# preiter93/rustpde-mpi

Hardware: NVIDIA H100
Metric: Navier2D timesteps/sec (higher is better)
Workload: dtype f64

## Files before the change

rustpde_mpi_b200/csrc/b200pde.cu:

```cuda
#include "lane_kernel.cuh"
#include "gemm_f64.cuh"
#include "../../include/b200pde.h"

#include <cmath>
#include <cstdlib>
#include <cstdio>
#include <cstring>
#include <map>
#include <string>
#include <vector>
#include <algorithm>

static thread_local std::string g_err;
static int fail(int code, const std::string& msg) { g_err = msg; return code; }
#define CK(call)                                                                                   \
  do {                                                                                             \
    cudaError_t e_ = (call);                                                                       \
    if (e_ != cudaSuccess)                                                                         \
      return fail(B2_ERR_CUDA, std::string(#call) + ": " + cudaGetErrorString(e_));                \
  } while (0)
#define RET(call)                    \
  do {                               \
    int r_ = (call);                 \
    if (r_ != B2_OK) return r_;      \
// ... 171 lines not shown
  LuVecs r;
  r.fl.assign(n, 0.0); r.id.assign(n, 0.0); r.u1.assign(n, 0.0); r.u2.assign(n, 0.0);
  for (int i = 0; i < n; i++) {
    if (i >= 2) r.fl[i] = low[i - 2];
    r.id[i] = 1.0 / dia[i];
    if (i < n - 2) r.u1[i] = up1[i];
    if (i < n - 4) r.u2[i] = up2[i];
  }
  return r;
}

static std::vector<double> pdma_sweep(int n, const std::vector<double> (&d)[7], int L) {
  const std::vector<double>&l2 = d[0], &l1 = d[1], &d0 = d[2], &u1 = d[3], &u2 = d[4], &u3 = d[5], &u4 = d[6];
  std::vector<double> al(n, 0.0), be(n, 0.0), ga(n, 0.0), de(n, 0.0), ka(n, 0.0), mu(n, 0.0);
  for (int i = 0; i < n; i++) {
    const double l2i = i >= 2 ? l2[i - 2] : 0.0;
    ka[i] = (i >= 1 ? l1[i - 1] : 0.0) - (i >= 2 ? al[i - 2] * l2i : 0.0);
    mu[i] = d0[i] - (i >= 2 ? be[i - 2] * l2i : 0.0) - (i >= 1 ? al[i - 1] * ka[i] : 0.0);
    if (i + 1 < n) al[i] = (u1[i] - (i >= 2 ? ga[i - 2] * l2i : 0.0) - (i >= 1 ? be[i - 1] * ka[i] : 0.0)) / mu[i];
    if (i + 2 < n) be[i] = (u2[i] - (i >= 2 ? de[i - 2] * l2i : 0.0) - (i >= 1 ? ga[i - 1] * ka[i] : 0.0)) / mu[i];
    if (i + 3 < n) ga[i] = (u3[i] - (i >= 1 ? de[i - 1] * ka[i] : 0.0)) / mu[i];
    if (i + 4 < n) de[i] = u4[i] / mu[i];
  }
  std::vector<double> out((size_t)7 * L, 0.0);
  for (int i = 0; i < n; i++) {
    out[i] = i >= 2 ? l2[i - 2] : 0.0; out[(size_t)L + i] = ka[i]; out[(size_t)2 * L + i] = 1.0 / mu[i];
    out[(size_t)3 * L + i] = al[i]; out[(size_t)4 * L + i] = be[i]; out[(size_t)5 * L + i] = ga[i]; out[(size_t)6 * L + i] = de[i];
  }
  return out;
}

static std::map<const void*, const void*>& scan_of() { static std::map<const void*, const void*> m; return m; }

struct Base1 {
  int kind = 0, n = 0, m = 0;
  bool cheb = false, composite = false;
  bool cdn = false;
  bool c2c = false;
  int rows_phys = 0, rows_spec = 0, rows_ortho = 0;
  int N = 0;
  std::vector<double> s2;
  DVecD d_sten2, d_sten2s, d_s2, d_tfl, d_tid, d_tu1, d_bd, d_bu1, d_bu2, d_tw, d_tw2, d_isin;
  std::vector<double> ca, cb;
  DVecD d_dfwd, d_dbwd; bool dense_tr = false;
  DVecD d_ca, d_cb, d_pent; int pent_L = 0;
  DVecD d_s2_sc, d_bd_sc, d_bu1_sc, d_bu2_sc, d_sten2s_sc;

  double pv(int i, int off) const {
    const int r = i + 2;
    if (off == 0) return r == 2 ? 0.25 : 1.0 / (4.0 * r * (r - 1.0));
    if (off == 2) return (r < n - 2) ? -1.0 / (2.0 * ((double)r * r - 1.0)) : 0.0;
    if (off == 4) return (r < n - 4) ? 1.0 / (4.0 * r * (r + 1.0)) : 0.0;
    return 0.0;
  }
  Diags mat_a() const {
    Diags a(m);
    for (int i = 0; i < m; i++) {
      if (i >= 2) a.low[i - 2] = pv(i, 0) * s2[i - 2];
      a.dia[i] = pv(i, 0) + pv(i, 2) * s2[i];
      if (i + 2 < m) a.up1[i] = pv(i, 2) + pv(i, 4) * s2[i + 2];
      if (i + 4 < m) a.up2[i] = pv(i, 4);
    }
    return a;
  }
  Diags mat_b() const {
    Diags b(m);
    for (int i = 0; i < m; i++) {
      b.dia[i] = s2[i];
      if (i + 2 < m) b.up1[i] = 1.0;
    }
    return b;
  }
  void cdn_hholtz_diags(double c, std::vector<double> (&d)[7]) const {
    auto S = [&](int r, int j) -> double { if (j < 0 || j >= m) return 0.0; return r == j ? 1.0 : (r == j + 1 ? ca[j] : (r == j + 2 ? cb[j] : 0.0)); };
    for (int k = 0; k < 7; k++) d[k].assign(m, 0.0);
    for (int i = 0; i < m; i++)
      for (int off = -2; off <= 4; off++) {
        const int j = i + off;
        if (j < 0 || j >= m) continue;
        const double a = pv(i, 0) * S(i, j) + pv(i, 2) * S(i + 2, j) + pv(i, 4) * S(i + 4, j);
        const double v = a - c * S(i + 2, j);
        d[off + 2][off >= 0 ? i : j] = v;
      }
  }
  int init_host(int kind_, int n_);
  int init(int C, int TPL);
  int lay_C = 1, lay_TPL = 1;
  std::vector<double> scan_layout(const std::vector<double>& v) const {
    std::vector<double> o((size_t)2 * lay_C * lay_TPL, 0.0);
    for (int q = 0; q < lay_TPL; q++)
      for (int t = 0; t < lay_C; t++) {
        const size_t p = (size_t)q * lay_C + t, k = (size_t)t * lay_TPL + q;
        if (2 * p < v.size()) o[2 * k] = v[2 * p];
        if (2 * p + 1 < v.size()) o[2 * k + 1] = v[2 * p + 1];
      }
    return o;
  }
  void release() {
    const void* keys[] = {d_bd.d, d_bu1.d, d_bu2.d, d_s2.d, d_sten2s.d};
    for (auto k : keys) if (k) scan_of().erase(k);
    DVecD* all[] = {&d_sten2, &d_sten2s, &d_s2, &d_tfl, &d_tid, &d_tu1, &d_bd, &d_bu1, &d_bu2, &d_tw, &d_tw2, &d_isin, &d_s2_sc, &d_bd_sc, &d_bu1_sc, &d_bu2_sc, &d_sten2s_sc, &d_ca, &d_cb, &d_pent, &d_dfwd, &d_dbwd};
    for (auto* v : all) v->release();
  }
};

static bool is_pow2(int x) { return x > 0 && (x & (x - 1)) == 0; }

int Base1::init_host(int kind_, int n_) {
  kind = kind_; n = n_;
  cheb = (kind <= B2_CHEB_DIRICHLET_NEUMANN);
  composite = (kind == B2_CHEB_DIRICHLET || kind == B2_CHEB_NEUMANN);
  cdn = (kind == B2_CHEB_DIRICHLET_NEUMANN);
  c2c = (kind == B2_FOURIER_C2C);
  if (kind < 0 || kind > B2_FOURIER_C2C) return fail(B2_ERR_ARG, "bad base kind");
  if (n < 5) return fail(B2_ERR_ARG, "n too small");
  if (cheb) {
    m = (composite || cdn) ? n - 2 : n;
    rows_phys = n; rows_spec = m; rows_ortho = n; N = n - 1;
  } else if (c2c) {
    if (n > 1024) return fail(B2_ERR_UNSUPPORTED, "fourier_c2c: n <= 1024 (dense-matrix transform)");
    m = n;
    rows_phys = 2 * n; rows_spec = 2 * n; rows_ortho = 2 * n; N = 0;
  } else {
    if (n % 2) return fail(B2_ERR_UNSUPPORTED, "fourier_r2c needs even n");
    m = n / 2 + 1;
    rows_phys = n; rows_spec = 2 * m; rows_ortho = 2 * m; N = n;
  }
  if (cdn) {
    ca.assign(m, 0.0); cb.assign(m, 0.0);
    for (int k = 0; k < m; k++) { const double kd = k; ca[k] = ((kd + 2) * (kd + 2) - kd * kd) / ((kd + 1) * (kd + 1) + (kd + 2) * (kd + 2)); cb[k] = ca[k] - 1.0; }
  }
  if (composite) {
    s2.assign(m, 0.0);
    for (int k = 0; k < m; k++) s2[k] = (kind == B2_CHEB_DIRICHLET) ? -1.0 : -((double)k / (k + 2.0)) * ((double)k / (k + 2.0));
  }
  return B2_OK;
}

int Base1::init(int C, int TPL) {
  lay_C = C; lay_TPL = TPL;
  const int L = roundup(std::max(rows_phys, rows_ortho) + 8, 4) + 64;
  if (composite) {
    std::vector<double> sten2(L, 0.0), s2v(L, 0.0);
    for (int i = 2; i < n; i++) sten2[i] = s2[i - 2];
    for (int k = 0; k < m; k++) s2v[k] = s2[k];
    RET(d_sten2.upload(sten2)); RET(d_sten2s.upload(sten2)); RET(d_s2.upload(s2v));
    Diags t(m);
    for (int k = 0; k < m; k++) {
      t.dia[k] = 1.0 + s2[k] * s2[k];
      if (k + 2 < m) { t.low[k] = s2[k]; t.up1[k] = s2[k]; }
    }
    LuVecs lu = sweep(t);
    lu.fl.resize(L, 0.0); lu.id.resize(L, 0.0); lu.u1.resize(L, 0.0);
    RET(d_tfl.upload(scan_layout(lu.fl))); RET(d_tid.upload(scan_layout(lu.id))); RET(d_tu1.upload(scan_layout(lu.u1)));
    std::vector<double> bd(L, 0.0), bu1(L, 0.0), bu2(L, 0.0);
    for (int i = 0; i < m; i++) {
      bd[i] = pv(i, 0);
      if (i < m - 2) bu1[i] = pv(i, 2);
      if (i < m - 4) bu2[i] = pv(i, 4);
    }
    RET(d_bd.upload(bd)); RET(d_bu1.upload(bu1)); RET(d_bu2.upload(bu2));
    RET(d_bd_sc.upload(scan_layout(bd))); RET(d_bu1_sc.upload(scan_layout(bu1))); RET(d_bu2_sc.upload(scan_layout(bu2))); RET(d_s2_sc.upload(scan_layout(s2v)));
    scan_of()[d_bd.d] = d_bd_sc.d; scan_of()[d_bu1.d] = d_bu1_sc.d; scan_of()[d_bu2.d] = d_bu2_sc.d; scan_of()[d_s2.d] = d_s2_sc.d;
    RET(d_sten2s_sc.upload(scan_layout(sten2))); scan_of()[d_sten2s.d] = d_sten2s_sc.d;
  }
  if (cdn) {
    std::vector<double> a(L, 0.0), b(L, 0.0);
    for (int k = 0; k < m; k++) { a[k] = ca[k]; b[k] = cb[k]; }
    RET(d_ca.upload(a)); RET(d_cb.upload(b));
    std::vector<double> d[7];
    for (int k = 0; k < 7; k++) d[k].assign(m, 0.0);
    for (int j = 0; j < m; j++) {
      d[2][j] = 1.0 + ca[j] * ca[j] + cb[j] * cb[j];
      if (j + 1 < m) { d[3][j] = ca[j] + cb[j] * ca[j + 1]; d[1][j] = d[3][j]; }
      if (j + 2 < m) { d[4][j] = cb[j]; d[0][j] = cb[j]; }
    }
    pent_L = L;
    RET(d_pent.upload(pdma_sweep(m, d, L)));
    std::vector<double> bd(L, 0.0), bu1(L, 0.0), bu2(L, 0.0);
    for (int i = 0; i < m; i++) {
      bd[i] = pv(i, 0);
      if (i < m - 2) bu1[i] = pv(i, 2);
      if (i < m - 4) bu2[i] = pv(i, 4);
    }
    RET(d_bd.upload(bd)); RET(d_bu1.upload(bu1)); RET(d_bu2.upload(bu2));
    RET(d_bd_sc.upload(scan_layout(bd))); RET(d_bu1_sc.upload(scan_layout(bu1))); RET(d_bu2_sc.upload(scan_layout(bu2)));
    scan_of()[d_bd.d] = d_bd_sc.d; scan_of()[d_bu1.d] = d_bu1_sc.d; scan_of()[d_bu2.d] = d_bu2_sc.d;
// ... 56 lines not shown
struct b2_space {
  b2_ctx* ctx = nullptr;
  Base1 b[2];
  int P[2] = {0, 0};
  PassCfg cfg[2];
  bool transforms_ok = false;
  size_t elems() const { return (size_t)P[0] * P[1] / ctx->nranks; }
  double* tmp[6] = {nullptr};
  int refs = 0;
};

struct b2_array {
  b2_space* sp;
  double* d;
  int shape_kind;
};

struct b2_field {
  b2_space* sp;
  b2_array* v;
  b2_array* vhat;
};

struct GemmPlan {
  DVecD A[2];
  GemmParams p;
  int grid = 0;
};

struct b2_solver {
  b2_space* sp = nullptr;
  int type = 0;
  DVecD fl[2], id[2], u1[2], u2[2], sd[2], pd[2];
  int pd_L[2] = {0, 0};
  bool dense = false;
  int m0 = 0;
  DVecD pfl, pid, pu1, pu2;
  bool blocks = false;
  int ce = 0, co = 0;
  DVecD qfl, qid, qu1, qu2;
  GemmPlan gf, gb;
  bool own_gemm = false;
};

__device__ __forceinline__ size_t tiled_index(int r, int c, int tiles) {
  return ((size_t)(r >> 2) * tiles + (c >> 2)) * 16 + (r & 3) * 4 + (c & 3);
}
__global__ void k_host_layout(double* tiled, double* plain, int rows, int cols, int tiles, int cplx, int to_tiled) {
  size_t idx = (size_t)blockIdx.x * blockDim.x + threadIdx.x;
  size_t total = (size_t)rows * cols;
  if (idx >= total) return;
  int r = (int)(idx / cols), c = (int)(idx % cols);
  size_t p = cplx ? (((size_t)(r >> 1) * cols + c) * 2 + (r & 1)) : idx;
  size_t t = tiled_index(r, c, tiles);
  if (to_tiled) tiled[t] = plain[p]; else plain[p] = tiled[t];
}
__global__ void k_axpby(size_t n, double* __restrict__ y, double a, const double* __restrict__ x, double b) {
  size_t i = (size_t)blockIdx.x * blockDim.x + threadIdx.x;
  size_t stride = (size_t)gridDim.x * blockDim.x;
  for (; i < n; i += stride) y[i] = a * x[i] + b * y[i];
}
__global__ void k_muladd(size_t n, double* __restrict__ out, const double* __restrict__ u, const double* __restrict__ p, int acc) {
  size_t i = (size_t)blockIdx.x * blockDim.x + threadIdx.x;
  size_t stride = (size_t)gridDim.x * blockDim.x;
  for (; i < n; i += stride) out[i] = (acc ? out[i] : 0.0) + u[i] * p[i];
}
// ... 164 lines not shown
  bool exchange = false;
  int npst = 0;
  if (ctx->nranks > 1) {
    for (int i = 0; i < p.nops; i++)
      if (p.ops[i].code == OP_STORE && (p.ops[i].i2 & ST_TRANS)) { p.ops[i].i2 |= ST_PEER; p.ops[i].p1 = ctx->d_peers; exchange = true; }
      else if (p.ops[i].code == OP_STORE && (p.ops[i].i2 & ST_COLSPLIT)) { p.ops[i].p1 = ctx->d_peers; exchange = true; }
  } else {
    for (int i = 0; i < p.nops; i++) if (p.ops[i].code == OP_STORE) p.ops[i].i2 &= ~ST_COLSPLIT;
  }
  for (int i = 0; !c.fast && i + 1 < p.nops; i++) {
    LaneOp& lo = p.ops[i]; LaneOp& bo = p.ops[i + 1];
    if (lo.code != OP_LOAD || (lo.i2 & (LD_PLAIN | LD_STENCIL | LD_ACC | LD_MUL)) || bo.code != OP_BAND) continue;
    const int h0 = (int)(signed char)(bo.i1 & 0xff), h1 = (int)(signed char)((bo.i1 >> 8) & 0xff), h2 = (int)(signed char)((bo.i1 >> 16) & 0xff);
    if (h0 != 0 || bo.p0 != nullptr || h1 != -2 || bo.p1 == nullptr || h2 != 127 || bo.i2 != lo.i0) continue;
    lo.i2 |= LD_STENCIL; lo.p1 = bo.p1; lo.i0 = bo.i0;
    bo.code = OP_PREBAND;
  }
  if (c.fast && c.E <= 8) {
    for (int i = 0; i + 1 < p.nops; i++) {
      LaneOp& bo = p.ops[i]; LaneOp& fo = p.ops[i + 1];
      if (bo.code != OP_BAND || fo.code != OP_FDMA || (fo.i2 & FD_PERLANE) || bo.i0 != fo.i0) continue;
      bool ok = true;
      const void* sc[3] = {nullptr, nullptr, nullptr};
      const void* nat[3] = {bo.p0, bo.p1, bo.p2};
      for (int m = 0; m < 3; m++) {
        const int h = (int)(signed char)((bo.i1 >> (8 * m)) & 0xff);
        if (h == 127) continue;
        if (h != 0 && h != 2 && h != 4) ok = false;
        if (nat[m]) { auto it = scan_of().find(nat[m]); if (it == scan_of().end()) ok = false; else sc[m] = it->second; }
      }
      if (!ok) continue;
      bo.code = OP_PREBAND; bo.p0 = sc[0]; bo.p1 = sc[1]; bo.p2 = sc[2]; fo.i2 |= FD_PREBAND;
    }
  }
  if (c.fast) {
    for (int i = 0; i < p.nops; i++) {
      LaneOp& bo = p.ops[i];
      if (bo.code != OP_BAND) continue;
      const void* nat[3] = {bo.p0, bo.p1, bo.p2};
      const void* slot[3] = {nullptr, nullptr, nullptr};
      int flag[3] = {0, 0, 0};
      bool ok = true, anyvec = false, fwd = false, bwd = false;
      for (int m = 0; m < 3 && ok; m++) {
        const int h = (int)(signed char)((bo.i1 >> (8 * m)) & 0xff);
        if (h == 127) continue;
        int k;
        if (h == 0) k = 0; else if (h == 2) { k = 1; fwd = true; } else if (h == 4) { k = 2; fwd = true; } else if (h == -2) { k = 1; bwd = true; } else { ok = false; break; }
        if (flag[k]) { ok = false; break; }
        if (nat[m]) { auto it = scan_of().find(nat[m]); if (it == scan_of().end()) { ok = false; break; } slot[k] = it->second; flag[k] = 2; anyvec = true; }
        else flag[k] = 1;
      }
      if (!ok || !anyvec || (fwd && bwd)) continue;
      bo.code = OP_BANDC; bo.p0 = slot[0]; bo.p1 = slot[1]; bo.p2 = slot[2];
      bo.i1 = (bwd ? 1 : 0) | (flag[0] << 2) | (flag[1] << 4) | (flag[2] << 6);
    }
  }
  const int groups_local = c.groups / ctx->nranks;
  for (int i = 0; i < p.nops && g_use_tma; i++) {
    LaneOp& op = p.ops[i];
    B2TMapDesc d; memset(&d, 0, sizeof(d));
    if (op.code == OP_LOAD && !(op.i2 & LD_PLAIN)) {
      const bool direct = !(op.i2 & (LD_ACC | LD_MUL | LD_STENCIL)) && op.a == 1.0;
      for (int k = 0; k < i; k++)
        if (p.ops[k].code == OP_STORE && p.ops[k].p0 == op.p0) op.i2 |= LD_AFTER_STORE;
      if (!direct && !g_use_ring) continue;
      d.base = const_cast<void*>(op.p0); d.rank = 3;
// ... 204 lines not shown
  RET(run_pass(sp, 0, y));
  Prog x; x.load(sp->tmp[0], b0.rows_ortho); l = x.from_ortho(b0); x.store(vhat, l, ST_TRANS | (acc ? ST_ACC : 0), alpha);
  return run_pass(sp, 1, x);
}
static int op_gradient(b2_space* sp, const double* vhat, int d0, int d1, const double* scale, double* out, double alpha = 1.0, bool acc = false) {
  const Base1& b0 = sp->b[0]; const Base1& b1 = sp->b[1];
  double s0 = 1.0, s1 = 1.0;
  if (scale) { s0 = 1.0 / std::pow(scale[0], d0); s1 = 1.0 / std::pow(scale[1], d1); }
  Prog y; y.load(vhat, b1.rows_spec); y.to_ortho(b1); int l = y.deriv_axis(b1, d1, s1); y.store(sp->tmp[0], l, ST_TRANS);
  RET(run_pass(sp, 0, y));
  Prog x; x.load(sp->tmp[0], b0.rows_spec); x.to_ortho(b0); l = x.deriv_axis(b0, d0, s0); x.store(out, l, ST_TRANS | (acc ? ST_ACC : 0), alpha);
  return run_pass(sp, 1, x);
}
static int op_backward_ortho(b2_space* sp, const double* ortho, double* phys) {
  const Base1& b0 = sp->b[0]; const Base1& b1 = sp->b[1];
  if (!sp->transforms_ok) return fail(B2_ERR_UNSUPPORTED, "transform size");
  Prog y; y.load(ortho, b1.rows_ortho); int l = y.backward_ortho(b1); y.store(sp->tmp[0], l, ST_TRANS);
  RET(run_pass(sp, 0, y));
  Prog x; x.load(sp->tmp[0], b0.rows_ortho); l = x.backward_ortho(b0); x.store(phys, l, ST_TRANS);
  return run_pass(sp, 1, x);
}
static int op_forward_ortho_dealias(b2_space* sp, const double* phys, double* ortho, bool dealias, double alpha = 1.0, bool acc = false) {
  const Base1& b0 = sp->b[0]; const Base1& b1 = sp->b[1];
  if (!sp->transforms_ok) return fail(B2_ERR_UNSUPPORTED, "transform size");
  const int shape0 = b0.cheb ? b0.n : b0.m, shape1 = b1.cheb ? b1.n : b1.m;
  const int cut0 = (shape0 * 2 / 3) * (b0.cheb ? 1 : 2), cut1 = (shape1 * 2 / 3) * (b1.cheb ? 1 : 2);
  Prog y; y.load(phys, b1.rows_phys); int l = y.forward_ortho(b1); if (dealias) y.zerotail(cut1); y.store(sp->tmp[0], l, ST_TRANS);
  RET(run_pass(sp, 0, y));
  Prog x; x.load(sp->tmp[0], b0.rows_phys); l = x.forward_ortho(b0); if (dealias) x.zerotail(cut0);
  x.store(ortho, l, ST_TRANS | (acc ? ST_ACC : 0), alpha);
  return run_pass(sp, 1, x);
}

static int upload_lu(const LuVecs& lu, const Base1& b, DVecD* fl, DVecD* id, DVecD* u1, DVecD* u2) {
  RET(fl->upload(b.scan_layout(lu.fl))); RET(id->upload(b.scan_layout(lu.id)));
  RET(u1->upload(b.scan_layout(lu.u1))); RET(u2->upload(b.scan_layout(lu.u2)));
  return B2_OK;
}

static int hholtz_create(b2_space* sp, double c0, double c1, b2_solver** out) {
  b2_solver* s = new b2_solver();
  s->sp = sp; s->type = 0;
  const double c[2] = {c0, c1};
  for (int ax = 0; ax < 2; ax++) {
    const Base1& b = sp->b[ax];
    const int L = sp->P[ax] + 64;
    if (b.composite) {
      Diags a = b.mat_a(), bm = b.mat_b(), mat(b.m);
      for (int i = 0; i < b.m; i++) {
        mat.low[i] = a.low[i] - bm.low[i] * c[ax];
        mat.dia[i] = a.dia[i] - bm.dia[i] * c[ax];
        mat.up1[i] = a.up1[i] - bm.up1[i] * c[ax];
        mat.up2[i] = a.up2[i] - bm.up2[i] * c[ax];
      }
      RET(upload_lu(sweep(mat), b, &s->fl[ax], &s->id[ax], &s->u1[ax], &s->u2[ax]));
    } else if (b.cdn) {
      std::vector<double> d[7];
      b.cdn_hholtz_diags(c[ax], d);
      s->pd_L[ax] = L;
      RET(s->pd[ax].upload(pdma_sweep(b.m, d, L)));
    } else if (!b.cheb) {
      std::vector<double> sd(L, 0.0);
      for (int k = 0; k < b.m; k++) {
        const double kk = (b.c2c && 2 * k >= b.n) ? k - b.n : k;
        sd[k] = 1.0 / (1.0 - (-kk * kk) * c[ax]);
      }
      RET(s->sd[ax].upload(sd));
    } else {
      delete s;
      return fail(B2_ERR_UNSUPPORTED, "HholtzAdi on an orthonormal Chebyshev axis is not on the Navier2D path");
    }
  }
  *out = s;
  return B2_OK;
}

static void emit_hh_axis(Prog& p, const b2_solver* s, int ax);
static int hholtz_solve(b2_solver* s, const double* in, double* out) {
  b2_space* sp = s->sp;
  const Base1& b0 = sp->b[0]; const Base1& b1 = sp->b[1];
  Prog y; y.load(in, b1.rows_ortho); emit_hh_axis(y, s, 1);
  y.store(sp->tmp[0], b1.rows_spec, ST_TRANS);
  RET(run_pass(sp, 0, y));
  Prog x; x.load(sp->tmp[0], b0.rows_ortho); emit_hh_axis(x, s, 0);
  x.store(out, b0.rows_spec, ST_TRANS);
  return run_pass(sp, 1, x);
}

// ... 599 lines not shown
  RET(need_kind(out, B2_SHAPE_ORTHO, "to_ortho"));
  return op_to_ortho(f->sp, f->vhat->d, out->d);
}
int b2_from_ortho(b2_field* f, const b2_array* in) {
  RET(need_kind(in, B2_SHAPE_ORTHO, "from_ortho"));
  return op_from_ortho(f->sp, in->d, f->vhat->d);
}
int b2_gradient(const b2_field* f, int d0, int d1, const double* scale, b2_array* out) {
  RET(need_kind(out, B2_SHAPE_ORTHO, "gradient"));
  if (d0 < 0 || d1 < 0 || d0 > 3 || d1 > 3) return fail(B2_ERR_ARG, "gradient: derivative order");
  return op_gradient(f->sp, f->vhat->d, d0, d1, scale, out->d);
}

int b2_field_dealias(b2_field* f) {
  b2_space* sp = f->sp;
  const Base1& b0 = sp->b[0]; const Base1& b1 = sp->b[1];
  if (b0.c2c) return fail(B2_ERR_UNSUPPORTED, "dealias: the 2/3 tail rule of functions.rs:72-82 is written for r2c / Chebyshev mode order");
  const int cut0 = (b0.m * 2 / 3) * (b0.cheb ? 1 : 2), cut1 = b1.m * 2 / 3;
  Prog y; y.load(f->vhat->d, b1.rows_spec); y.zerotail(cut1); y.store(sp->tmp[0], b1.rows_spec, ST_TRANS);
  RET(run_pass(sp, 0, y));
  Prog x; x.load(sp->tmp[0], b0.rows_spec); x.zerotail(cut0); x.store(f->vhat->d, b0.rows_spec, ST_TRANS);
  return run_pass(sp, 1, x);
}

int b2_hholtz_adi_create(const b2_field* f, double c0, double c1, b2_solver** out) { return hholtz_create(f->sp, c0, c1, out); }
int b2_poisson_create(const b2_field* f, double c0, double c1, const double* lam, const double* fwd, const double* bwd, b2_solver** out) {
  return poisson_create(f->sp, c0, c1, lam, fwd, bwd, out);
}
int b2_hholtz_create(const b2_field* f, double c0, double c1, const double* lam, const double* fwd, const double* bwd, b2_solver** out) {
  return poisson_create(f->sp, c0, c1, lam, fwd, bwd, out, true);
}
int b2_solver_destroy(b2_solver* s) {
  if (!s) return B2_OK;
  for (int ax = 0; ax < 2; ax++) { s->fl[ax].release(); s->id[ax].release(); s->u1[ax].release(); s->u2[ax].release(); s->sd[ax].release(); s->pd[ax].release(); }
  s->pfl.release(); s->pid.release(); s->pu1.release(); s->pu2.release();
  s->qfl.release(); s->qid.release(); s->qu1.release(); s->qu2.release();
  for (GemmPlan* g : {&s->gf, &s->gb}) { g->A[0].release(); g->A[1].release(); }
  delete s;
  return B2_OK;
}
int b2_solve(b2_solver* s, const b2_array* in, b2_array* out) {
  RET(need_kind(in, B2_SHAPE_ORTHO, "solve input"));
  RET(need_kind(out, B2_SHAPE_SPECTRAL, "solve output"));
  if (in->sp != s->sp || out->sp != s->sp) return fail(B2_ERR_SHAPE, "solve: arrays belong to a different space");
  return s->type == 0 ? hholtz_solve(s, in->d, out->d) : poisson_solve(s, in->d, out->d, false);
}

static void dense_from_diags(const Diags& d, double* out) {
  const int m = d.m;
  std::fill(out, out + (size_t)m * m, 0.0);
  for (int i = 0; i < m; i++) {
    out[(size_t)i * m + i] = d.dia[i];
    if (i + 2 < m) { out[(size_t)(i + 2) * m + i] = d.low[i]; out[(size_t)i * m + i + 2] = d.up1[i]; }
    if (i + 4 < m) out[(size_t)i * m + i + 4] = d.up2[i];
  }
}
int b2_host_poisson_matrices(int kind0, int n0, double c0, double* a0, double* cmat0) {
  Base1 b0;
  RET(b0.init_host(kind0, n0));
  if (!b0.composite) return fail(B2_ERR_ARG, "axis 0 is not a composite Chebyshev base");
  Diags lap, mass;
  poisson_axis(b0, c0, &lap, &mass);
  dense_from_diags(lap, a0);
  dense_from_diags(mass, cmat0);
  return B2_OK;
}
int b2_poisson_axis0_matrices(const b2_field* f, double c0, double* a0, double* cmat0) {
// ... 405 lines not shown
```

rustpde_mpi_b200/csrc/lane_fast.cuh:

```cuda
#pragma once

template <int LN, int K> struct POff { static_assert(K % 2 == 0, "even pair offsets only"); static constexpr int v = (K / 2) * (1 << Lay<LN>::LSH); };
template <int LN, int K> struct EOff { static_assert(K % 4 == 0, "element offsets in tiles only"); static constexpr int v = (K / 4) * (1 << (Lay<LN>::LSH + 1)); };

template <int E, int R, int Ns, int LN, int TPL, bool SWZI, bool SWZO>
__device__ __forceinline__ void fstage(double2* __restrict__ wl, int q, const cplx* __restrict__ tw) {
  constexpr int NB = E / R, LE = Log2<E>::v, Nc = E * TPL, stride = Nc / R, LSH = Lay<LN>::LSH;
  constexpr int RS = POff<LN, stride>::v;
  static_assert(!SWZI || stride % (1 << LE) == 0, "swizzled reads need stride to be a multiple of E");
  cplx v[E];
  cplx w1[NB];
#pragma unroll
  for (int b = 0; b < NB; b++) {
    const int j = q + b * TPL;
    if (Ns > 1) w1[b] = ldg(tw + (j & (Ns - 1)) * (stride / Ns));
    if (!SWZI) {
      const int base = Lay<LN>::pix(j);
#pragma unroll
      for (int r = 0; r < R; r++) v[b * R + r] = wl[base + r * RS];
    } else {
      const int s0 = (j >> LE) & 1;
      const int b0 = Lay<LN>::pix(j ^ s0), b1 = Lay<LN>::pix(j ^ (s0 ^ 1));
#pragma unroll
      for (int r = 0; r < R; r++) v[b * R + r] = wl[(((r * (stride >> LE)) & 1) ? b1 : b0) + r * RS];
// ... 313 lines not shown
  const int p0 = q * CP;
  const ChunkAddr<LN> ca(p0);
  const int tmax = HP - p0;
  for (int rep = 0; rep < op.i1; rep++) {
    double2 tp[CP];
    double2 tot = d2(0.0, 0.0);
#pragma unroll
    for (int t = 0; t < CP; t++) {
      const bool ok = t < tmax;
      const double2 a = ok ? w2[ca.at(t)] : d2(0.0, 0.0);
      const double f = 4.0 * (p0 + t);
      tp[t] = d2(f * a.x, (f + 2.0) * a.y);
      tot.x += tp[t].x; tot.y += tp[t].y;
    }
    Aff1::V m; m.d[0] = 1; m.d[1] = tot.x; m.d[2] = 1; m.d[3] = tot.y;
    Aff1::S in = lane_scan_state<Aff1, true, LN>(m, TPL, scratch);
    double2 S = d2(in.d[0], in.d[1]);
    const double sc = (rep == op.i1 - 1) ? op.a : 1.0;
#pragma unroll
    for (int t = CP - 1; t >= 0; t--) {
      const double nx = S.x;
      S.x += tp[t].x; S.y += tp[t].y;
      double2 o = d2(S.y * sc, nx * sc);
      if (t == 0 && q == 0) o.x *= 0.5;
      if (t < tmax) w2[ca.at(t)] = o;
    }
    __syncthreads();
  }
}

template <int E, int LN, int TPL, bool PERLANE, bool PREBAND>
__device__ __forceinline__ void fdma_fast_body(const LaneProg& P, const LaneOp& op, double* __restrict__ W, int gl, int lb, void* scratch) {
  constexpr int CP = E + 1, CS = PERLANE ? 4 * TPL : TPL;
  const int HP = P.LP >> 1;
  const int l = threadIdx.x & (LN - 1), q = threadIdx.x >> Lay<LN>::LOG;
  const int n = op.i0;
  double2* w2 = reinterpret_cast<double2*>(W) + 2 * l;
  const size_t cb = PERLANE ? ((size_t)gl * CP * TPL + q) * 4 + lb + l : (size_t)q;
  const double2* __restrict__ cfl = (const double2*)op.p0 + cb; const double2* __restrict__ cid = (const double2*)op.p1 + cb;
  const double2* __restrict__ cu1 = (const double2*)op.p2 + cb; const double2* __restrict__ cu2 = (const double2*)op.p3 + cb;
  const bool nou2 = op.i2 & FD_NOU2;
  const double2 zero = d2(0.0, 0.0);
  const int p0 = q * CP;
  const ChunkAddr<LN> ca(p0);
  const int tmax = HP - p0;
  const int tx = (n - 2 * p0 + 1) >> 1, ty = (n - 2 * p0) >> 1;
  const bool interior = (tmax >= CP) && (ty >= CP);
  auto rdm = [&](int t) -> double2 {
    double2 v = (t < tmax) ? w2[ca.at(t)] : zero;
    if (t >= tx) v.x = 0.0;
    if (t >= ty) v.y = 0.0;
    return v;
  };
  PhaseClock pc(P.prof);
  {
    double2 A = d2(1.0, 1.0), B = zero;
    if constexpr (PREBAND) {
      const LaneOp& bop = *(&op - 1);
      const double2* cf[3] = {cfl, cfl, cfl};
      double wl[3] = {0.0, 0.0, 0.0}, ad[3] = {0.0, 0.0, 0.0};
#pragma unroll
      for (int m = 0; m < 3; m++) {
        const int h = (int)(signed char)((bop.i1 >> (8 * m)) & 0xff);
        const double2* cp = (const double2*)(m == 0 ? bop.p0 : (m == 1 ? bop.p1 : bop.p2));
#pragma unroll
        for (int k = 0; k < 3; k++)
          if (h == 2 * k) { if (cp) { cf[k] = cp + q; wl[k] = 1.0; } else ad[k] = 1.0; }
      }
      const double2 hA = (CP < tmax) ? w2[ca.at(CP)] : zero, hB = (CP + 1 < tmax) ? w2[ca.at(CP + 1)] : zero;
      __syncthreads();
      double2 x0 = (0 < tmax) ? w2[ca.at(0)] : zero, x1 = (1 < tmax) ? w2[ca.at(1)] : zero;
#pragma unroll
      for (int t = 0; t < CP; t++) {
        const double2 x2 = (t + 2 < CP) ? ((t + 2 < tmax) ? w2[ca.at(t + 2 < CP ? t + 2 : 0)] : zero) : (t + 2 == CP ? hA : hB);
        double2 b = zero;
        const double2 l0 = ldg(cf[0] + t * TPL), l1 = ldg(cf[1] + t * TPL), l2 = ldg(cf[2] + t * TPL);
        const double2 k0 = d2(fma(l0.x, wl[0], ad[0]), fma(l0.y, wl[0], ad[0]));
        const double2 k1 = d2(fma(l1.x, wl[1], ad[1]), fma(l1.y, wl[1], ad[1]));
        const double2 k2 = d2(fma(l2.x, wl[2], ad[2]), fma(l2.y, wl[2], ad[2]));
        b = d2fma(k0, x0, d2fma(k1, x1, d2(k2.x * x2.x, k2.y * x2.y)));
        if (t >= tx) b.x = 0.0;
        if (t >= ty) b.y = 0.0;
        if (t < tmax) w2[ca.at(t)] = b;
        const double2 f = ldg(cfl + t * CS);
        B = d2(fma(-f.x, B.x, b.x), fma(-f.y, B.y, b.y));
        A = d2(-f.x * A.x, -f.y * A.y);
        x0 = x1; x1 = x2;
      }
    } else if (interior) {
#pragma unroll
      for (int t = 0; t < CP; t++) {
        const double2 f = ldg(cfl + t * CS), b = w2[ca.at(t)];
        B = d2(fma(-f.x, B.x, b.x), fma(-f.y, B.y, b.y));
        A = d2(-f.x * A.x, -f.y * A.y);
      }
    } else {
#pragma unroll
      for (int t = 0; t < CP; t++) {
        const double2 f = ldg(cfl + t * CS), b = rdm(t);
        B = d2(fma(-f.x, B.x, b.x), fma(-f.y, B.y, b.y));
        A = d2(-f.x * A.x, -f.y * A.y);
      }
    }
    pc.mark(16);
    Aff1::V m; m.d[0] = A.x; m.d[1] = B.x; m.d[2] = A.y; m.d[3] = B.y;
    Aff1::S in = lane_scan_state<Aff1, false, LN>(m, TPL, scratch);
    pc.mark(17);
    double2 y = d2(in.d[0], in.d[1]);
    if (interior) {
#pragma unroll
      for (int t = 0; t < CP; t++) {
        const double2 f = ldg(cfl + t * CS), b = w2[ca.at(t)];
        y = d2(fma(-f.x, y.x, b.x), fma(-f.y, y.y, b.y));
        w2[ca.at(t)] = y;
      }
    } else {
#pragma unroll
      for (int t = 0; t < CP; t++) {
        const double2 f = ldg(cfl + t * CS), b = rdm(t);
        y = d2(fma(-f.x, y.x, b.x), fma(-f.y, y.y, b.y));
        if (t < tmax) w2[ca.at(t)] = y;
      }
    }
  }
  pc.mark(18);
  {
    Aff2::V m = Aff2::identity();
    auto compose = [&](int t, double2 y) {
      const double2 idv = ldg(cid + t * CS), u1 = ldg(cu1 + t * CS), u2 = nou2 ? zero : ldg(cu2 + t * CS);
      const double2 m0 = d2(-u1.x * idv.x, -u1.y * idv.y), m1 = d2(-u2.x * idv.x, -u2.y * idv.y), g0 = d2(y.x * idv.x, y.y * idv.y);
      double* Mx = m.d;
      double r0 = m0.x * Mx[0] + m1.x * Mx[2], r1 = m0.x * Mx[1] + m1.x * Mx[3], rp = m0.x * Mx[4] + m1.x * Mx[5] + g0.x;
      Mx[2] = Mx[0]; Mx[3] = Mx[1]; Mx[5] = Mx[4]; Mx[0] = r0; Mx[1] = r1; Mx[4] = rp;
      Mx = m.d + 6;
      r0 = m0.y * Mx[0] + m1.y * Mx[2]; r1 = m0.y * Mx[1] + m1.y * Mx[3]; rp = m0.y * Mx[4] + m1.y * Mx[5] + g0.y;
      Mx[2] = Mx[0]; Mx[3] = Mx[1]; Mx[5] = Mx[4]; Mx[0] = r0; Mx[1] = r1; Mx[4] = rp;
    };
    if (interior) {
#pragma unroll
      for (int t = CP - 1; t >= 0; t--) compose(t, w2[ca.at(t)]);
    } else {
#pragma unroll
      for (int t = CP - 1; t >= 0; t--) compose(t, rdm(t));
    }
    pc.mark(19);
    Aff2::S in = lane_scan_state<Aff2, true, LN>(m, TPL, scratch);
    pc.mark(20);
    double2 s1 = d2(in.d[0], in.d[2]), s2 = d2(in.d[1], in.d[3]);
    auto solve = [&](int t, double2 y) -> double2 {
      const double2 idv = ldg(cid + t * CS), u1 = ldg(cu1 + t * CS), u2 = nou2 ? zero : ldg(cu2 + t * CS);
      const double2 x = d2((y.x - u1.x * s1.x - u2.x * s2.x) * idv.x, (y.y - u1.y * s1.y - u2.y * s2.y) * idv.y);
      s2 = s1; s1 = x;
      return x;
    };
    if (interior) {
#pragma unroll
      for (int t = CP - 1; t >= 0; t--) w2[ca.at(t)] = solve(t, w2[ca.at(t)]);
    } else {
#pragma unroll
      for (int t = CP - 1; t >= 0; t--) { const double2 x = solve(t, rdm(t)); if (t < tmax) w2[ca.at(t)] = x; }
    }
  }
  __syncthreads();
  pc.mark(21);
}
template <int E, int LN, int TPL>
__device__ __noinline__ void fdma_fast(const LaneProg& P, const LaneOp& op, double* __restrict__ W, int gl, int lb, void* scratch) {
  if (op.i2 & FD_PERLANE) fdma_fast_body<E, LN, TPL, true, false>(P, op, W, gl, lb, scratch);
  else if (op.i2 & FD_PREBAND) fdma_fast_body<E, LN, TPL, false, true>(P, op, W, gl, lb, scratch);
  else fdma_fast_body<E, LN, TPL, false, false>(P, op, W, gl, lb, scratch);
}
```

rustpde_mpi_b200/csrc/lane_kernel.cuh:

```cuda
#pragma once
#ifdef B2_EMU
#include "cuda_emu.h"
#else
#include <cuda_runtime.h>
#define B2_DYN_SMEM(type, name) extern __shared__ __align__(1024) type name[]
#define B2_LAUNCH(kernel, grid, block, smem, stream, ...) kernel<<<(grid), (block), (smem), (stream)>>>(__VA_ARGS__)
#endif
#include <stdint.h>
#include <stddef.h>
#include "async_ops.cuh"

#define B2_MAXOPS 24
#define B2_MAXPEERS 8
#define B2_MAXPST 6
#define B2_BARBYTES 512
#define B2_SCRATCH 8192
#define B2_PROGCOPY 2048

enum LaneOpCode {
  OP_LOAD = 1,
  OP_STORE = 2,
  OP_BAND = 3,
  OP_DERIV = 4,
  OP_FDMA = 5,
  OP_DCT = 6,
  OP_RFFT = 7,
  OP_FDIFF = 8,
  OP_SCALEVEC = 9,
  OP_ZEROTAIL = 10,
  OP_LANEMASK = 11,
  OP_ZEROELEM = 12,
  OP_SCALE = 13,
  OP_PREBAND = 14,
  OP_BANDC = 15,
  OP_STEN3 = 16,
  OP_DENSE = 18,
  OP_PDMA = 17,
};
enum { LD_ACC = 1, LD_PLAIN = 2, LD_MUL = 4, LD_STENCIL = 8,
       LD_TMA = 16,
       LD_AFTER_STORE = 32,
       LD_DIRECT = 64,
       LD_PSPLIT = 128,
       LD_PSPLITC = 256 };
enum { ST_ACC = 1, ST_PLAIN = 2, ST_TRANS = 8, ST_PEER = 16,
       ST_TMA = 32,
       ST_DIRECT = 64,
       ST_PSPLIT = 128,
       ST_PSPLITC = 256,
       ST_COLSPLIT = 512 };
enum { FD_PERLANE = 1, FD_NOU2 = 2,
       FD_PREBAND = 4 };

struct LaneOp {
  int code, i0, i1, i2;
  double a, b;
  const void* p0;
  const void* p1;
  const void* p2;
  const void* p3;
};

struct LaneProg {
  int nops;
  int LP;
  int in_tiles;
  int out_tiles;
  int TPL;
  int C;
  int group0;
  int groups_per_rank;
  int rank;
  int LN;
  int NT;
  int CHW, nsc;
  int wslot_bytes;
  int CHD, nchd;
  int w_off, st_off;
  int bulk1d;
  unsigned long long* prof;
  LaneOp ops[B2_MAXOPS];
  B2TMap tm[B2_MAXOPS];
  B2TMap tmp[B2_MAXPST][B2_MAXPEERS];
};

// ... 1092 lines not shown
```

Measured before the change: 63.74.

## Precompute per-chunk LU affine maps on host to shorten lane-parallel FDMA scans

Adds a host-side table, computed in long double, holding per-chunk LU solve data: the product of forward factors, the composed 2x2 backward transfer matrix, and weight vectors that turn the backward affine offset into dot products. The fast FDMA kernel now reads these constants from one interleaved table. This replaces the serial per-element matrix composition in the backward pass and the running product in the forward pass, and folds id into u1/u2 so the back-substitution becomes FMAs. The intent is to cut dependent FLOPs in the lane-parallel tridiagonal/pentadiagonal scan. The cost is more table loads, extra setup memory, and a hard failure when no table exists for the lane layout.

Measured after the change: 65.92 (median of 6 runs). 3.4% higher.

```diff
diff --git a/rustpde_mpi_b200/csrc/b200pde.cu b/rustpde_mpi_b200/csrc/b200pde.cu
--- a/rustpde_mpi_b200/csrc/b200pde.cu
+++ b/rustpde_mpi_b200/csrc/b200pde.cu
@@ -227,6 +227,46 @@
 
 static std::map<const void*, const void*>& scan_of() { static std::map<const void*, const void*> m; return m; }
 
+struct LuMapRef { const void* table; int C, TPL; };
+static std::map<const void*, LuMapRef>& lumap_of() { static std::map<const void*, LuMapRef> m; return m; }
+
+static std::vector<double> lu_chunk_maps(const std::vector<double>& fl, const std::vector<double>& id, const std::vector<double>& u1,
+                                         const std::vector<double>* u2, int C, int TPL) {
+  const int NS = LM_CHUNK * C + LMC_N;
+  std::vector<double> o((size_t)2 * NS * TPL, 0.0);
+  std::vector<long double> wa(C), wb(C);
+  for (int q = 0; q < TPL; q++)
+    for (int h = 0; h < 2; h++) {
+      auto in = [&](const std::vector<double>& v, int t) -> long double { return v[((size_t)t * TPL + q) * 2 + h]; };
+      auto out = [&](int s) -> double& { return o[((size_t)s * TPL + q) * 2 + h]; };
+      long double A = 1.0L, P00 = 1.0L, P01 = 0.0L, P10 = 0.0L, P11 = 1.0L;
+      for (int t = 0; t < C; t++) {
+        const long double u2t = u2 ? in(*u2, t) : 0.0L;
+        out(LM_FL * C + t) = (double)in(fl, t); out(LM_ID * C + t) = (double)in(id, t);
+        out(LM_U1 * C + t) = (double)(in(u1, t) * in(id, t)); out(LM_U2 * C + t) = (double)(u2t * in(id, t));
+        A *= -in(fl, t);
+      }
+      for (int t = C - 1; t >= 0; t--) {
+        const long double m0 = -in(u1, t) * in(id, t), m1 = -(u2 ? in(*u2, t) : 0.0L) * in(id, t);
+        for (int k = t + 1; k < C; k++) { const long double a = wa[k]; wa[k] = m0 * a + m1 * wb[k]; wb[k] = a; }
+        wa[t] = in(id, t); wb[t] = 0.0L;
+        const long double r0 = m0 * P00 + m1 * P10, r1 = m0 * P01 + m1 * P11;
+        P10 = P00; P11 = P01; P00 = r0; P01 = r1;
+      }
+      for (int t = 0; t < C; t++) { out(LM_WA * C + t) = (double)wa[t]; out(LM_WB * C + t) = (double)wb[t]; }
+      out(LM_CHUNK * C + LMC_A) = (double)A;
+      out(LM_CHUNK * C + LMC_P + 0) = (double)P00; out(LM_CHUNK * C + LMC_P + 1) = (double)P01;
+      out(LM_CHUNK * C + LMC_P + 2) = (double)P10; out(LM_CHUNK * C + LMC_P + 3) = (double)P11;
+    }
+  return o;
+}
+static int upload_lu_maps(const void* fl_key, const std::vector<double>& fl, const std::vector<double>& id, const std::vector<double>& u1,
+                          const std::vector<double>* u2, int C, int TPL, DVecD* table) {
+  RET(table->upload(lu_chunk_maps(fl, id, u1, u2, C, TPL)));
+  lumap_of()[fl_key] = LuMapRef{table->d, C, TPL};
+  return B2_OK;
+}
+
 struct Base1 {
   int kind = 0, n = 0, m = 0;
   bool cheb = false, composite = false;
@@ -240,6 +280,7 @@
   DVecD d_dfwd, d_dbwd; bool dense_tr = false;
   DVecD d_ca, d_cb, d_pent; int pent_L = 0;
   DVecD d_s2_sc, d_bd_sc, d_bu1_sc, d_bu2_sc, d_sten2s_sc;
+  DVecD d_tmap;
 
   double pv(int i, int off) const {
     const int r = i + 2;
@@ -294,7 +335,8 @@
   void release() {
     const void* keys[] = {d_bd.d, d_bu1.d, d_bu2.d, d_s2.d, d_sten2s.d};
     for (auto k : keys) if (k) scan_of().erase(k);
-    DVecD* all[] = {&d_sten2, &d_sten2s, &d_s2, &d_tfl, &d_tid, &d_tu1, &d_bd, &d_bu1, &d_bu2, &d_tw, &d_tw2, &d_isin, &d_s2_sc, &d_bd_sc, &d_bu1_sc, &d_bu2_sc, &d_sten2s_sc, &d_ca, &d_cb, &d_pent, &d_dfwd, &d_dbwd};
+    if (d_tfl.d) lumap_of().erase(d_tfl.d);
+    DVecD* all[] = {&d_sten2, &d_sten2s, &d_s2, &d_tfl, &d_tid, &d_tu1, &d_bd, &d_bu1, &d_bu2, &d_tw, &d_tw2, &d_isin, &d_s2_sc, &d_bd_sc, &d_bu1_sc, &d_bu2_sc, &d_sten2s_sc, &d_ca, &d_cb, &d_pent, &d_dfwd, &d_dbwd, &d_tmap};
     for (auto* v : all) v->release();
   }
 };
@@ -347,7 +389,9 @@
     }
     LuVecs lu = sweep(t);
     lu.fl.resize(L, 0.0); lu.id.resize(L, 0.0); lu.u1.resize(L, 0.0);
-    RET(d_tfl.upload(scan_layout(lu.fl))); RET(d_tid.upload(scan_layout(lu.id))); RET(d_tu1.upload(scan_layout(lu.u1)));
+    const std::vector<double> tfl = scan_layout(lu.fl), tid = scan_layout(lu.id), tu1 = scan_layout(lu.u1);
+    RET(d_tfl.upload(tfl)); RET(d_tid.upload(tid)); RET(d_tu1.upload(tu1));
+    RET(upload_lu_maps(d_tfl.d, tfl, tid, tu1, nullptr, C, TPL, &d_tmap));
     std::vector<double> bd(L, 0.0), bu1(L, 0.0), bu2(L, 0.0);
     for (int i = 0; i < m; i++) {
       bd[i] = pv(i, 0);
@@ -470,6 +514,7 @@
   b2_space* sp = nullptr;
   int type = 0;
   DVecD fl[2], id[2], u1[2], u2[2], sd[2], pd[2];
+  DVecD lm[2];
   int pd_L[2] = {0, 0};
   bool dense = false;
   int m0 = 0;
@@ -700,6 +745,14 @@
       if (!ok) continue;
       bo.code = OP_PREBAND; bo.p0 = sc[0]; bo.p1 = sc[1]; bo.p2 = sc[2]; fo.i2 |= FD_PREBAND;
     }
+  }
+  for (int i = 0; c.fast && i < p.nops; i++) {
+    LaneOp& fo = p.ops[i];
+    if (fo.code != OP_FDMA || (fo.i2 & FD_PERLANE)) continue;
+    const auto it = lumap_of().find(fo.p0);
+    if (it == lumap_of().end() || it->second.C != c.C || it->second.TPL != c.TPL)
+      return fail(B2_ERR_ARG, "LU solve without a chunk-map table for this lane layout");
+    fo.p0 = it->second.table;
   }
   if (c.fast) {
     for (int i = 0; i < p.nops; i++) {
@@ -970,10 +1023,10 @@
   return run_pass(sp, 1, x);
 }
 
-static int upload_lu(const LuVecs& lu, const Base1& b, DVecD* fl, DVecD* id, DVecD* u1, DVecD* u2) {
-  RET(fl->upload(b.scan_layout(lu.fl))); RET(id->upload(b.scan_layout(lu.id)));
-  RET(u1->upload(b.scan_layout(lu.u1))); RET(u2->upload(b.scan_layout(lu.u2)));
-  return B2_OK;
+static int upload_lu(const LuVecs& lu, const Base1& b, DVecD* fl, DVecD* id, DVecD* u1, DVecD* u2, DVecD* map) {
+  const std::vector<double> sfl = b.scan_layout(lu.fl), sid = b.scan_layout(lu.id), su1 = b.scan_layout(lu.u1), su2 = b.scan_layout(lu.u2);
+  RET(fl->upload(sfl)); RET(id->upload(sid)); RET(u1->upload(su1)); RET(u2->upload(su2));
+  return upload_lu_maps(fl->d, sfl, sid, su1, &su2, b.lay_C, b.lay_TPL, map);
 }
 
 static int hholtz_create(b2_space* sp, double c0, double c1, b2_solver** out) {
@@ -991,7 +1044,7 @@
         mat.up1[i] = a.up1[i] - bm.up1[i] * c[ax];
         mat.up2[i] = a.up2[i] - bm.up2[i] * c[ax];
       }
-      RET(upload_lu(sweep(mat), b, &s->fl[ax], &s->id[ax], &s->u1[ax], &s->u2[ax]));
+      RET(upload_lu(sweep(mat), b, &s->fl[ax], &s->id[ax], &s->u1[ax], &s->u2[ax], &s->lm[ax]));
     } else if (b.cdn) {
       std::vector<double> d[7];
       b.cdn_hholtz_diags(c[ax], d);
@@ -1657,7 +1710,10 @@
 }
 int b2_solver_destroy(b2_solver* s) {
   if (!s) return B2_OK;
-  for (int ax = 0; ax < 2; ax++) { s->fl[ax].release(); s->id[ax].release(); s->u1[ax].release(); s->u2[ax].release(); s->sd[ax].release(); s->pd[ax].release(); }
+  for (int ax = 0; ax < 2; ax++) {
+    if (s->fl[ax].d) lumap_of().erase(s->fl[ax].d);
+    s->fl[ax].release(); s->id[ax].release(); s->u1[ax].release(); s->u2[ax].release(); s->sd[ax].release(); s->pd[ax].release(); s->lm[ax].release();
+  }
   s->pfl.release(); s->pid.release(); s->pu1.release(); s->pu2.release();
   s->qfl.release(); s->qid.release(); s->qu1.release(); s->qu2.release();
   for (GemmPlan* g : {&s->gf, &s->gb}) { g->A[0].release(); g->A[1].release(); }
diff --git a/rustpde_mpi_b200/csrc/lane_fast.cuh b/rustpde_mpi_b200/csrc/lane_fast.cuh
--- a/rustpde_mpi_b200/csrc/lane_fast.cuh
+++ b/rustpde_mpi_b200/csrc/lane_fast.cuh
@@ -369,13 +369,16 @@
 template <int E, int LN, int TPL, bool PERLANE, bool PREBAND>
 __device__ __forceinline__ void fdma_fast_body(const LaneProg& P, const LaneOp& op, double* __restrict__ W, int gl, int lb, void* scratch) {
   constexpr int CP = E + 1, CS = PERLANE ? 4 * TPL : TPL;
+  constexpr bool MAPS = !PERLANE;
   const int HP = P.LP >> 1;
   const int l = threadIdx.x & (LN - 1), q = threadIdx.x >> Lay<LN>::LOG;
   const int n = op.i0;
   double2* w2 = reinterpret_cast<double2*>(W) + 2 * l;
   const size_t cb = PERLANE ? ((size_t)gl * CP * TPL + q) * 4 + lb + l : (size_t)q;
-  const double2* __restrict__ cfl = (const double2*)op.p0 + cb; const double2* __restrict__ cid = (const double2*)op.p1 + cb;
-  const double2* __restrict__ cu1 = (const double2*)op.p2 + cb; const double2* __restrict__ cu2 = (const double2*)op.p3 + cb;
+  const double2* __restrict__ cfl = (const double2*)op.p0 + cb;
+  const double2* __restrict__ cid = MAPS ? cfl + LM_ID * CP * TPL : (const double2*)op.p1 + cb;
+  const double2* __restrict__ cu1 = MAPS ? cfl + LM_U1 * CP * TPL : (const double2*)op.p2 + cb;
+  const double2* __restrict__ cu2 = MAPS ? cfl + LM_U2 * CP * TPL : (const double2*)op.p3 + cb;
   const bool nou2 = op.i2 & FD_NOU2;
   const double2 zero = d2(0.0, 0.0);
   const int p0 = q * CP;
@@ -390,6 +393,9 @@
     return v;
   };
   PhaseClock pc(P.prof);
+  double2 ta = zero, tb = zero;
+  const double2* __restrict__ cwa = cfl + LM_WA * CP * TPL;
+  const double2* __restrict__ cwb = cfl + LM_WB * CP * TPL;
   {
     double2 A = d2(1.0, 1.0), B = zero;
     if constexpr (PREBAND) {
@@ -421,7 +427,7 @@
         if (t < tmax) w2[ca.at(t)] = b;
         const double2 f = ldg(cfl + t * CS);
         B = d2(fma(-f.x, B.x, b.x), fma(-f.y, B.y, b.y));
-        A = d2(-f.x * A.x, -f.y * A.y);
+        if constexpr (!MAPS) A = d2(-f.x * A.x, -f.y * A.y);
         x0 = x1; x1 = x2;
       }
     } else if (interior) {
@@ -429,16 +435,17 @@
       for (int t = 0; t < CP; t++) {
         const double2 f = ldg(cfl + t * CS), b = w2[ca.at(t)];
         B = d2(fma(-f.x, B.x, b.x), fma(-f.y, B.y, b.y));
-        A = d2(-f.x * A.x, -f.y * A.y);
+        if constexpr (!MAPS) A = d2(-f.x * A.x, -f.y * A.y);
       }
     } else {
 #pragma unroll
       for (int t = 0; t < CP; t++) {
         const double2 f = ldg(cfl + t * CS), b = rdm(t);
         B = d2(fma(-f.x, B.x, b.x), fma(-f.y, B.y, b.y));
-        A = d2(-f.x * A.x, -f.y * A.y);
-      }
-    }
+        if constexpr (!MAPS) A = d2(-f.x * A.x, -f.y * A.y);
+      }
+    }
+    if constexpr (MAPS) A = ldg(cfl + (LM_CHUNK * CP + LMC_A) * TPL);
     pc.mark(16);
     Aff1::V m; m.d[0] = A.x; m.d[1] = B.x; m.d[2] = A.y; m.d[3] = B.y;
     Aff1::S in = lane_scan_state<Aff1, false, LN>(m, TPL, scratch);
@@ -450,6 +457,7 @@
         const double2 f = ldg(cfl + t * CS), b = w2[ca.at(t)];
         y = d2(fma(-f.x, y.x, b.x), fma(-f.y, y.y, b.y));
         w2[ca.at(t)] = y;
+        if constexpr (MAPS) { ta = d2fma(ldg(cwa + t * TPL), y, ta); tb = d2fma(ldg(cwb + t * TPL), y, tb); }
       }
     } else {
 #pragma unroll
@@ -457,28 +465,41 @@
         const double2 f = ldg(cfl + t * CS), b = rdm(t);
         y = d2(fma(-f.x, y.x, b.x), fma(-f.y, y.y, b.y));
         if (t < tmax) w2[ca.at(t)] = y;
+        if constexpr (MAPS) {
+          double2 v = (t < tmax) ? y : zero;
+          if (t >= tx) v.x = 0.0;
+          if (t >= ty) v.y = 0.0;
+          ta = d2fma(ldg(cwa + t * TPL), v, ta); tb = d2fma(ldg(cwb + t * TPL), v, tb);
+        }
       }
     }
   }
   pc.mark(18);
   {
     Aff2::V m = Aff2::identity();
-    auto compose = [&](int t, double2 y) {
-      const double2 idv = ldg(cid + t * CS), u1 = ldg(cu1 + t * CS), u2 = nou2 ? zero : ldg(cu2 + t * CS);
-      const double2 m0 = d2(-u1.x * idv.x, -u1.y * idv.y), m1 = d2(-u2.x * idv.x, -u2.y * idv.y), g0 = d2(y.x * idv.x, y.y * idv.y);
-      double* Mx = m.d;
-      double r0 = m0.x * Mx[0] + m1.x * Mx[2], r1 = m0.x * Mx[1] + m1.x * Mx[3], rp = m0.x * Mx[4] + m1.x * Mx[5] + g0.x;
-      Mx[2] = Mx[0]; Mx[3] = Mx[1]; Mx[5] = Mx[4]; Mx[0] = r0; Mx[1] = r1; Mx[4] = rp;
-      Mx = m.d + 6;
-      r0 = m0.y * Mx[0] + m1.y * Mx[2]; r1 = m0.y * Mx[1] + m1.y * Mx[3]; rp = m0.y * Mx[4] + m1.y * Mx[5] + g0.y;
-      Mx[2] = Mx[0]; Mx[3] = Mx[1]; Mx[5] = Mx[4]; Mx[0] = r0; Mx[1] = r1; Mx[4] = rp;
-    };
-    if (interior) {
-#pragma unroll
-      for (int t = CP - 1; t >= 0; t--) compose(t, w2[ca.at(t)]);
-    } else {
-#pragma unroll
-      for (int t = CP - 1; t >= 0; t--) compose(t, rdm(t));
+    if constexpr (MAPS) {
+      const double2* __restrict__ cP = cfl + (LM_CHUNK * CP + LMC_P) * TPL;
+      const double2 P00 = ldg(cP), P01 = ldg(cP + TPL), P10 = ldg(cP + 2 * TPL), P11 = ldg(cP + 3 * TPL);
+      m.d[0] = P00.x; m.d[1] = P01.x; m.d[2] = P10.x; m.d[3] = P11.x; m.d[4] = ta.x; m.d[5] = tb.x;
+      m.d[6] = P00.y; m.d[7] = P01.y; m.d[8] = P10.y; m.d[9] = P11.y; m.d[10] = ta.y; m.d[11] = tb.y;
+    } else {
+      auto compose = [&](int t, double2 y) {
+        const double2 idv = ldg(cid + t * CS), u1 = ldg(cu1 + t * CS), u2 = nou2 ? zero : ldg(cu2 + t * CS);
+        const double2 m0 = d2(-u1.x * idv.x, -u1.y * idv.y), m1 = d2(-u2.x * idv.x, -u2.y * idv.y), g0 = d2(y.x * idv.x, y.y * idv.y);
+        double* Mx = m.d;
+        double r0 = m0.x * Mx[0] + m1.x * Mx[2], r1 = m0.x * Mx[1] + m1.x * Mx[3], rp = m0.x * Mx[4] + m1.x * Mx[5] + g0.x;
+        Mx[2] = Mx[0]; Mx[3] = Mx[1]; Mx[5] = Mx[4]; Mx[0] = r0; Mx[1] = r1; Mx[4] = rp;
+        Mx = m.d + 6;
+        r0 = m0.y * Mx[0] + m1.y * Mx[2]; r1 = m0.y * Mx[1] + m1.y * Mx[3]; rp = m0.y * Mx[4] + m1.y * Mx[5] + g0.y;
+        Mx[2] = Mx[0]; Mx[3] = Mx[1]; Mx[5] = Mx[4]; Mx[0] = r0; Mx[1] = r1; Mx[4] = rp;
+      };
+      if (interior) {
+#pragma unroll
+        for (int t = CP - 1; t >= 0; t--) compose(t, w2[ca.at(t)]);
+      } else {
+#pragma unroll
+        for (int t = CP - 1; t >= 0; t--) compose(t, rdm(t));
+      }
     }
     pc.mark(19);
     Aff2::S in = lane_scan_state<Aff2, true, LN>(m, TPL, scratch);
@@ -486,7 +507,8 @@
     double2 s1 = d2(in.d[0], in.d[2]), s2 = d2(in.d[1], in.d[3]);
     auto solve = [&](int t, double2 y) -> double2 {
       const double2 idv = ldg(cid + t * CS), u1 = ldg(cu1 + t * CS), u2 = nou2 ? zero : ldg(cu2 + t * CS);
-      const double2 x = d2((y.x - u1.x * s1.x - u2.x * s2.x) * idv.x, (y.y - u1.y * s1.y - u2.y * s2.y) * idv.y);
+      const double2 x = MAPS ? d2(fma(-u1.x, s1.x, fma(-u2.x, s2.x, idv.x * y.x)), fma(-u1.y, s1.y, fma(-u2.y, s2.y, idv.y * y.y)))
+                             : d2((y.x - u1.x * s1.x - u2.x * s2.x) * idv.x, (y.y - u1.y * s1.y - u2.y * s2.y) * idv.y);
       s2 = s1; s1 = x;
       return x;
     };
diff --git a/rustpde_mpi_b200/csrc/lane_kernel.cuh b/rustpde_mpi_b200/csrc/lane_kernel.cuh
--- a/rustpde_mpi_b200/csrc/lane_kernel.cuh
+++ b/rustpde_mpi_b200/csrc/lane_kernel.cuh
@@ -51,6 +51,8 @@
        ST_COLSPLIT = 512 };
 enum { FD_PERLANE = 1, FD_NOU2 = 2,
        FD_PREBAND = 4 };
+enum { LM_FL = 0, LM_ID, LM_U1, LM_U2, LM_WA, LM_WB, LM_CHUNK };
+enum { LMC_A = 0, LMC_P = 1, LMC_N = 5 };
 
 struct LaneOp {
   int code, i0, i1, i2;
```
